# omerbt/Splice

Measured on AMD Instinct MI355X. Metric: opt_steps_per_sec, higher is better.
Workload: dtype bf16

## Files before the change

### splice_amd/csrc/step_engine.hip

```cpp
#include <memory>
#include <vector>

#include <stdio.h>
#include <stdlib.h>
#include <string.h>

#include "gen_kernels.h"
#include "kernels.h"
#include "optim.h"
#include "plateau.h"
#include "step_graph.h"

enum { L_TOTAL = 0, L_GLOBAL_SSIM = 1, L_ENTIRE_SSIM = 2, L_ENTIRE_CLS = 3, L_GLOBAL_CLS = 4, L_GLOBAL_ID = 5, L_TERMS = 6 };
enum { LAM_CLS = 0, LAM_SSIM = 1, LAM_ID = 2, LAM_ECLS = 3, LAM_ESSIM = 4 };
enum { PW_ESCALE_G = 0, PW_ESCALE_E = 1, PW_CLS = 2, PW_ID = 3, PW_ECLS = 4, PW_LAMBDAS = 5, PW_ROWS = 10 };
static const int TERM_LAM[L_TERMS] = {-1, LAM_SSIM, LAM_ESSIM, LAM_ECLS, LAM_CLS, LAM_ID};
static const int TERM_ROW[L_TERMS] = {-1, PW_ESCALE_G, PW_ESCALE_E, PW_ECLS, PW_CLS, PW_ID};

struct VitView {
    void* ctx = nullptr;
    int B = 0, H = 0, W = 0, D = 0, depth = 0, heads = 0, patch = 0, T = 0, Tld = 0, rows = 0;
    float* d_block = nullptr;
    float* d_keys = nullptr;
    float* imgs = nullptr;
    float* d_imgs = nullptr;
    std::vector<const float*> pb, pk;
};

struct SpliceStep {
    splice_step_config cfg;
    int P = 1;
    int Pa = 1, Pb = 1;
    int crops_mode = 0;
    int pairs = 1;
    int na = 1, nb = 1;
    size_t astride = 0;
    VitView vg, ve;
    void *plan_a = nullptr, *plan_b = nullptr, *plan_e = nullptr;
    int cropb_h = 0, cropb_w = 0;
    long long nparams = 0;
    float* gen_in = nullptr;
    float* in_b = nullptr;
    float* ent_in = nullptr;
    float* gen_out = nullptr;
    float* gen_out_b = nullptr;
    float *d_gen_out = nullptr, *d_gen_out_b = nullptr;
    float* ent_out = nullptr;
    float* d_ent_out = nullptr;
    void* ssim_ws = nullptr;
    float* losses = nullptr;
    size_t lp = 0, lstride = 0;
    std::vector<void*> allocs;
    int max_crop_h = 0, max_crop_w = 0;
    int* dev_t = nullptr;
    float* dev_lr = nullptr;
    int lr_set = 0;
    float lr = 0.f;
    int opt_kind = SPLICE_OPT_ADAM;
    float* pw = nullptr;
    float* pw_tab_alloc = nullptr;
    int pw_any[5] = {0, 0, 0, 0, 0};
    float* dev_lrs = nullptr;
    int pair_lr = 0;
    float lrs[SPLICE_STEP_MAX_PAIR_CFGS] = {};
    float opt_hp0 = 0.f, opt_hp1 = 0.f, opt_eps = 0.f;
    hipStream_t own_stream = nullptr;
    enum { EV_IN, EV_OUT, EV_FORK, EV_JOIN, EV_GB, EV_FORK2, EV_JOIN2, EV_KINDS };
    static constexpr int EV_RING = 4;
    hipEvent_t evs[EV_RING][EV_KINDS] = {};
    int ev_slot = 0;
    hipEvent_t ev(int kind) const { return evs[ev_slot][kind]; }
    hipStream_t side_stream = nullptr;
    int overlap = 1;
    int ablate = 0;
    StepGraphs graphs;
    void* graph_ptrs[6] = {nullptr, nullptr, nullptr, nullptr, nullptr, nullptr};
    float* losses_out = nullptr;
    int graph_crops[4] = {0, 0, 0, 0};
    float* grads_b = nullptr;
    int shape_repeats = 0;
    int repeat_step = -1;
    int use_graph = 1;
    int dbg_sync = 0;
    int ssim_id_on = 0;
    int skip_adam = 0, accumulate = 0;
    float* running = nullptr;
    long long running_stride = 0;
    int phases = 7;
    SpliceStep* leader = nullptr;
    splice_stop_state* stop = nullptr;
    StopRule stop_rule = {0, 0.f, 0, 0};
    int runs = 0;
};

static size_t arena_floats(const SpliceStep* st) { return st->astride ? st->pairs * st->astride : (size_t)st->nparams; }
static bool create_events(SpliceStep* st) {
    for (auto& set : st->evs)
        for (hipEvent_t& e : set)
            if (hipEventCreateWithFlags(&e, hipEventDisableTiming) != hipSuccess) return false;
    return true;
}

template <class T>
static int salloc(SpliceStep* st, T** p, size_t n) {
    void* q = nullptr;
    if (hipMalloc(&q, n * sizeof(T) + 256) != hipSuccess) {
        splice_set_error("splice_step: hipMalloc of %zu bytes failed", n * sizeof(T));
        return SPLICE_ERR_NOMEM;
    }
    st->allocs.push_back(q);
    *p = (T*)q;
    return SPLICE_OK;
}

static int view_init(SpliceStep* st, VitView& v, void* ctx, int want_B) {
    v.ctx = ctx;
    RC(splice_vit_ctx_dims(ctx, &v.B, &v.H, &v.W, &v.D, &v.depth, &v.heads, &v.patch));
    RC(splice_vit_ctx_info(ctx, &v.T, &v.Tld, &v.rows));
    RC(splice_vit_ctx_set_top_cls_only(ctx, st->cfg.top_cls_only));
    if (v.B != want_B) { splice_set_error("splice_step_create: ViT context has batch %d, need %d", v.B, want_B); return SPLICE_ERR_ARG; }
    RC(salloc(st, &v.d_block, (size_t)v.rows * v.D));
    RC(salloc(st, &v.d_keys, (size_t)v.rows * v.D));
    RC(salloc(st, &v.imgs, (size_t)v.B * 3 * v.H * v.W));
    RC(salloc(st, &v.d_imgs, (size_t)v.B * 3 * v.H * v.W));
    if (hipMemset(v.d_block, 0, (size_t)v.rows * v.D * sizeof(float)) != hipSuccess || hipMemset(v.d_keys, 0, (size_t)v.rows * v.D * sizeof(float)) != hipSuccess)
        return SPLICE_ERR_HIP;
    v.pb.assign(v.depth, nullptr);
    v.pk.assign(v.depth, nullptr);
    v.pb[v.depth - 1] = v.d_block;
    v.pk[v.depth - 1] = v.d_keys;
    return SPLICE_OK;
}

template <bool MONITOR>
__global__ __launch_bounds__(320) void total_loss_kernel(float* lbase, size_t lstride, int lp, float w_ssim, float w_essim, float w_ecls, float w_cls,
                                                         float w_id, float* out8, int n_a, int n_b, int n_c, int n_e, const float* wtab, int ssim_on,
                                                         int entire, splice_stop_state* stop, const int* dev_t, StopRule rule) {
    __shared__ float raw[8];
    float* l = lbase + (size_t)blockIdx.x * lstride;
    const int k = 1 + (threadIdx.x >> 6), lane = threadIdx.x & 63;
    const int n_slots = k == L_GLOBAL_SSIM ? n_a : k == L_GLOBAL_ID ? n_b : k == L_GLOBAL_CLS ? n_c : n_e;
    const float* lp0 = lbase + (size_t)blockIdx.x * n_slots * lstride;
    float tot = 0.f;
    for (int slot = 0; slot < n_slots; ++slot) {
        const float* part = lp0 + (size_t)slot * lstride + 8 + (size_t)k * lp;
        float acc = 0.f;
        for (int i = lane; i < lp; i += 64) acc += part[i];
        tot += wave_sum(acc);
    }
    const float acc = tot;
// ... 292 lines not shown
    const int P = st->P;
    for (int i = 0; i < 5 * P; ++i)
        if (!(lambdas[i] >= 0.f)) { splice_set_error("splice_step_set_pair_weights: lambdas must be >= 0"); return SPLICE_ERR_ARG; }
    std::vector<float> t((size_t)PW_ROWS * P, 0.f);
    const VitView &vg = st->vg, &ve = st->ve;
    const float ls_g = 1.0f / ((float)vg.T * (float)vg.T);
    const float ls_e = st->plan_e ? 1.0f / ((float)ve.T * (float)ve.T) : 0.f;
    const size_t n_cls = (size_t)1 * vg.D, n_id = (size_t)vg.T * vg.D, n_ecls = (size_t)1 * ve.D;
    for (int k = 0; k < 5; ++k) st->pw_any[k] = 0;
    for (int p = 0; p < P; ++p) {
        const float* l = lambdas + (size_t)p * 5;
        for (int k = 0; k < 5; ++k) st->pw_any[k] |= l[k] > 0.f;
        t[PW_ESCALE_G * P + p] = 4.0f * l[LAM_SSIM] * ls_g;
        if (st->plan_e) t[PW_ESCALE_E * P + p] = 4.0f * l[LAM_ESSIM] * ls_e;
        t[PW_CLS * P + p] = l[LAM_CLS] / (float)n_cls;
        t[PW_ID * P + p] = l[LAM_ID] / (float)n_id;
        if (st->plan_e) t[PW_ECLS * P + p] = l[LAM_ECLS] / (float)n_ecls;
        for (int k = 0; k < 5; ++k) t[PW_LAMBDAS * P + (size_t)p * 5 + k] = l[k];
    }
    st->graphs.retire();
    HIPCHK(hipDeviceSynchronize());
    HIPCHK(hipMemcpy(st->pw_tab_alloc, t.data(), t.size() * sizeof(float), hipMemcpyHostToDevice));
    st->pw = st->pw_tab_alloc;
    return SPLICE_OK;
}
int splice_step_set_pair_lr(void* h, const float* lr) {
    SpliceStep* st = (SpliceStep*)h;
    RC(pair_cfgs_ok(st, lr, "splice_step_set_pair_lr"));
    if (st->astride % 4) { splice_set_error("splice_step_set_pair_lr: the arena stride must be a multiple of 4"); return SPLICE_ERR_ARG; }
    if (!st->pair_lr) st->graphs.retire();
    st->pair_lr = 1;
    for (int p = 0; p < st->P; ++p) st->lrs[p] = lr[p];
    return SPLICE_OK;
}
int splice_step_set_phases(void* h, int phases, void* leader) {
    SpliceStep* st = (SpliceStep*)h;
    if (!st || phases <= 0 || phases > 7 || leader == h || (leader && phases != 2) || (leader && ((SpliceStep*)leader)->leader)) return SPLICE_ERR_ARG;
    if ((phases != 7 || leader) && st->stop_rule.window > 0) { splice_set_error("splice_step_set_phases: a handle with a stop rule runs whole steps (no phase mode)"); return SPLICE_ERR_STATE; }
    if (st->leader != (SpliceStep*)leader) st->graphs.retire();
    st->phases = phases;
    st->leader = (SpliceStep*)leader;
    return SPLICE_OK;
}

int splice_step_set_stop_rule(void* h, int window, float rel, int patience, int min_steps) {
    SpliceStep* st = (SpliceStep*)h;
    if (!st) return SPLICE_ERR_ARG;
    if (!stop_rule_ok(window, rel, patience, min_steps, "splice_step_set_stop_rule")) return SPLICE_ERR_ARG;
    if (st->runs > 0) { splice_set_error("splice_step_set_stop_rule: the rule is set before the first step"); return SPLICE_ERR_STATE; }
    if (st->skip_adam || st->phases != 7 || st->leader) {
        splice_set_error("splice_step_set_stop_rule: not on a handle in gradient-only (splice_step_set_mode) or phase mode (splice_step_set_phases)");
        return SPLICE_ERR_STATE;
    }
    if ((window > 0) != (st->stop_rule.window > 0)) st->graphs.retire();
    st->stop_rule = StopRule{window, rel, patience, min_steps};
    return SPLICE_OK;
}
int splice_step_stop_state(void* h, splice_stop_state* out, splice_stream_t stream) {
    SpliceStep* st = (SpliceStep*)h;
    if (!st || !out) return SPLICE_ERR_ARG;
    HIPCHK(hipMemcpyAsync(out, st->stop, (size_t)st->pairs * sizeof(splice_stop_state), hipMemcpyDeviceToHost, (hipStream_t)stream));
    HIPCHK(hipStreamSynchronize((hipStream_t)stream));
    return SPLICE_OK;
}
int splice_plateau_update(splice_stop_state* state, const float* losses8, int pairs, int window, float rel, int patience, int min_steps, int step_idx,
                          int counted, splice_stream_t stream) {
    if (!state || !losses8 || pairs < 1 || step_idx < 0) return SPLICE_ERR_ARG;
    if (!stop_rule_ok(window, rel, patience, min_steps, "splice_plateau_update")) return SPLICE_ERR_ARG;
    if (!counted || window == 0) return SPLICE_OK;
    SPLICE_LAUNCH(plateau_update_kernel, dim3((pairs + 63) / 64), dim3(64), 0, (hipStream_t)stream, state, losses8, pairs, StopRule{window, rel, patience, min_steps}, step_idx);
    return SPLICE_OK;
}

int splice_step_set_running_stats(void* h, float* running, long long stride) {
    SpliceStep* st = (SpliceStep*)h;
    if (!st || (running && st->P > 1 && stride <= 0)) return SPLICE_ERR_ARG;
    st->running = running; st->running_stride = stride;
    return SPLICE_OK;
}

static int place_passes(VitView& v, const float* src, int h, int w, int pass, int n, hipStream_t s) {
    return place_images(src, h, w, v.imgs + (size_t)pass * 3 * v.H * v.W, v.H, v.W, n, s);
}
static int zero_seeds(VitView& v, int pass, int n, hipStream_t s) {
    const size_t passD = (size_t)v.Tld * v.D;
    RC(dev_zero_launch(v.d_block + pass * passD, n * passD * sizeof(float), s));
    return dev_zero_launch(v.d_keys + pass * passD, n * passD * sizeof(float), s);
}

static int step_body(SpliceStep* st, float* params, float* grads, float* m, float* v, bool ssim_on, bool entire, hipStream_t s) {
    const splice_step_config& c = st->cfg;
    VitView &vg = st->vg, &ve = st->ve;
    const int P = st->P, Pa = st->Pa, Pb = st->Pb, pairs = st->pairs;
    const int nc = st->na < st->nb ? st->na : st->nb, Pc = pairs * nc;
    Term t[L_TERMS] = {};
    step_terms(st, ssim_on, entire, t);
    const StepPtrs ip = step_ptrs(st);
    const StepPtrs src = st->leader ? step_ptrs(st->leader) : ip;
    const bool do_gf = (st->phases & 1) != 0, do_v = (st->phases & 2) != 0, do_gb = (st->phases & 4) != 0;
    const bool gen_fwd = do_gf && !(st->ablate & 1), gen_bwd = do_gb && !(st->ablate & 2);
    auto chain_bwd = [&](VitView& vw, int p0, int p1, bool vit, float* d_img, int h, int w, float* d_lead, void* plan, float* arena, int accumulate,
                         bool gen, hipStream_t q) -> int {
        if (do_v) {
            if (vit) RC(splice_vit_backward(vw.ctx, p0, p1, vw.pb.data(), nullptr, vw.pk.data(), vw.d_imgs, 1, q));
            RC(unplace_grads(vw.d_imgs + (size_t)p0 * 3 * vw.H * vw.W, vw.H, vw.W, d_img, h, w, p1 - p0, q));
            if (st->leader) RC(add_f32_launch(d_lead, d_img, (size_t)(p1 - p0) * 3 * h * w, q));
        }
        if (gen) RC(splice_gen_backward(plan, params, d_img, arena, accumulate, q));
        return SPLICE_OK;
    };
    const int pA = 0, pB = Pa, pX = Pa + Pb, pY = 2 * Pa + Pb, pEnd = 2 * (Pa + Pb);
    const bool overlap = st->overlap && !splice_prof_active();
    hipStream_t s2 = overlap ? st->side_stream : s;
    if (overlap) {
        HIPCHK(hipEventRecord(st->ev(SpliceStep::EV_FORK), s));
        HIPCHK(hipStreamWaitEvent(s2, st->ev(SpliceStep::EV_FORK), 0));
    }
    if (gen_fwd) {
        RC(splice_gen_forward_borrowed(st->plan_b, params, src.b_in, ip.y, s2));
        if (overlap) HIPCHK(hipEventRecord(st->ev(SpliceStep::EV_GB), s2));
    }
    float *blk_g = nullptr, *qkv_g = nullptr;
    RC(splice_vit_get_tensor(vg.ctx, 0, vg.depth - 1, (void**)&blk_g));
    RC(splice_vit_get_tensor(vg.ctx, 3, vg.depth - 1, (void**)&qkv_g));
    const size_t passD = (size_t)vg.Tld * vg.D;
    SelfSimBatch sb = {};
    if (do_v) {
        RC(place_passes(vg, src.a_in, c.crop_h, c.crop_w, pA, Pa, s2));
        RC(place_passes(vg, src.b_in, st->cropb_h, st->cropb_w, pB, Pb, s2));
        if (!(st->ablate & 8)) RC(splice_vit_forward_passes(vg.ctx, vg.imgs, 1, pX, pA, pX, s2));
        RC(dev_zero_launch(st->losses, (size_t)P * st->lstride * sizeof(float), s2));
        RC(zero_seeds(vg, pX, Pa + Pb, s2));
        if (t[L_GLOBAL_SSIM].on) {
            RC(ssim_batch(st, vg, pA, pX, Pa, t[L_GLOBAL_SSIM], L_GLOBAL_SSIM, &sb));
            RC(selfsim_target_launch(sb, s2));
        }
    }
    if (overlap) HIPCHK(hipEventRecord(st->ev(SpliceStep::EV_JOIN), s2));
    if (gen_fwd) {
        RC(splice_gen_forward_borrowed(st->plan_a, params, src.a_in, ip.x, s));
        if (overlap) HIPCHK(hipStreamWaitEvent(s, st->ev(SpliceStep::EV_GB), 0));
    }
    if (do_v) {
        RC(place_passes(vg, src.x, c.crop_h, c.crop_w, pX, Pa, s));
        RC(place_passes(vg, src.y, st->cropb_h, st->cropb_w, pY, Pb, s));
        if (!(st->ablate & 16)) RC(splice_vit_forward_passes(vg.ctx, vg.imgs, 1, pX, pX, pEnd, s));
    }
    if (overlap) HIPCHK(hipStreamWaitEvent(s, st->ev(SpliceStep::EV_JOIN), 0));
    if (do_v) {
        if (t[L_GLOBAL_SSIM].on) RC(selfsim_loss_launch(sb, s));
        if (t[L_GLOBAL_CLS].on) {
            if (pairs > 1 && st->na != st->nb) {
                for (int i = 0; i < nc; ++i)
                    RC(mse_batched_launch(blk_g + (pX + i) * passD, vg.D, st->na * passD, blk_g + (pB + i) * passD, vg.D, st->nb * passD, 1, vg.D, 1.0f,
                                          t[L_GLOBAL_CLS].lambda, loss_part(st, L_GLOBAL_CLS) + (size_t)i * st->lstride, (size_t)nc * st->lstride,
                                          vg.d_block + (pX + i) * passD, vg.D, st->na * passD, pairs, s, nullptr));
            } else {
                RC(mse_batched_launch(blk_g + pX * passD, vg.D, passD, blk_g + pB * passD, vg.D, passD, 1, vg.D, 1.0f, t[L_GLOBAL_CLS].lambda,
                                      loss_part(st, L_GLOBAL_CLS), st->lstride, vg.d_block + pX * passD, vg.D, passD, Pc, s, t[L_GLOBAL_CLS].tab));
            }
        }
        if (t[L_GLOBAL_ID].on)
            RC(mse_batched_launch(keys_ptr(vg, qkv_g, pY), 3 * vg.D, 3 * passD, keys_ptr(vg, qkv_g, pB), 3 * vg.D, 3 * passD, vg.T, vg.D, 1.0f, t[L_GLOBAL_ID].lambda,
                                  loss_part(st, L_GLOBAL_ID), st->lstride, vg.d_keys + pY * passD, vg.D, passD, Pb, s, t[L_GLOBAL_ID].tab));
    }
    if (entire) {
        if (do_gf) RC(splice_gen_forward_borrowed(st->plan_e, params, src.e_in, ip.xe, s));
        if (do_v) {
            RC(place_passes(ve, src.e_in, c.ent_h, c.ent_w, 0, pairs, s));
            RC(place_passes(ve, src.xe, c.ent_h, c.ent_w, pairs, pairs, s));
            RC(splice_vit_forward_ex(ve.ctx, ve.imgs, 1, pairs, s));
            float* blk_e = nullptr;
            RC(splice_vit_get_tensor(ve.ctx, 0, ve.depth - 1, (void**)&blk_e));
            const size_t epassD = (size_t)ve.Tld * ve.D;
            RC(zero_seeds(ve, pairs, pairs, s));
            if (t[L_ENTIRE_SSIM].on) {
                SelfSimBatch se = {};
                RC(ssim_batch(st, ve, 0, pairs, pairs, t[L_ENTIRE_SSIM], L_ENTIRE_SSIM, &se));
                RC(selfsim_target_launch(se, s));
                RC(selfsim_loss_launch(se, s));
            }
            if (t[L_ENTIRE_CLS].on)
                RC(mse_batched_launch(blk_e + pairs * epassD, ve.D, epassD, blk_g + pB * passD, vg.D, st->nb * passD, 1, ve.D, 1.0f, t[L_ENTIRE_CLS].lambda,
                                      loss_part(st, L_ENTIRE_CLS), st->lstride, ve.d_block + pairs * epassD, ve.D, epassD, pairs, s, t[L_ENTIRE_CLS].tab));
        }
    }
    const bool stop_on = st->stop_rule.window > 0;
    auto bookkeeping = [&](hipStream_t q) -> int {
        if (do_v) {
            const bool grouped = st->crops_mode && pairs > 1;
            const int n1 = st->crops_mode ? P : 1;
            const auto kernel = stop_on ? total_loss_kernel<true> : total_loss_kernel<false>;
            SPLICE_LAUNCH(kernel, dim3(pairs), dim3(320), 0, q, st->losses, st->lstride, (int)st->lp, t[L_GLOBAL_SSIM].lambda, t[L_ENTIRE_SSIM].lambda,
                          t[L_ENTIRE_CLS].lambda, t[L_GLOBAL_CLS].lambda, t[L_GLOBAL_ID].lambda, st->losses_out, grouped ? st->na : n1, grouped ? st->nb : n1, grouped ? nc : n1,
                          grouped ? 1 : n1, st->pw ? st->pw + (size_t)PW_LAMBDAS * P : nullptr, (int)ssim_on, (int)entire, st->stop, st->dev_t, st->stop_rule);
        }
        if (!st->running || !gen_fwd) return SPLICE_OK;
        void* plans[3] = {st->plan_a, st->plan_b, nullptr};
        if (entire) { plans[1] = st->plan_e; plans[2] = st->plan_b; }
        return gen_running_stats_update(plans, entire ? 3 : 2, st->running, st->running_stride, 0.1f, stop_on ? st->stop : nullptr, st->dev_t, q);
    };
    const bool side_tail = overlap && !(st->ablate & 4);
    const float* adam_g2 = nullptr;
    if (!(st->ablate & 4)) {
        if (overlap) {
            HIPCHK(hipEventRecord(st->ev(SpliceStep::EV_FORK2), s));
            HIPCHK(hipStreamWaitEvent(s2, st->ev(SpliceStep::EV_FORK2), 0));
        }
        RC(chain_bwd(vg, pY, pEnd, !(st->ablate & 32), ip.dy, st->cropb_h, st->cropb_w, src.dy, st->plan_b, st->grads_b, 0, gen_bwd, s2));
        if (side_tail) {
            RC(bookkeeping(s2));
            HIPCHK(hipEventRecord(st->ev(SpliceStep::EV_JOIN2), s2));
        }
        RC(chain_bwd(vg, pX, pY, true, ip.dx, c.crop_h, c.crop_w, src.dx, st->plan_a, grads, st->accumulate, gen_bwd, s));
        if (overlap) HIPCHK(hipStreamWaitEvent(s, st->ev(SpliceStep::EV_JOIN2), 0));
        if (gen_bwd) {
            if (entire || st->skip_adam) RC(add_f32_launch(grads, st->grads_b, arena_floats(st), s));
            else adam_g2 = st->grads_b;
        }
    }
    if (entire) RC(chain_bwd(ve, pairs, 2 * pairs, true, ip.dxe, c.ent_h, c.ent_w, src.dxe, st->plan_e, grads, 1, do_gb, s));
    if (!side_tail) RC(bookkeeping(s));
    SPLICE_DEV_REGION(21);
    if (do_gb && !st->skip_adam) {
        OptimArgs a = {};
        a.kind = st->opt_kind; a.p = params; a.g = grads; a.g2 = adam_g2; a.m = m; a.v = v;
        a.n = arena_floats(st);
        a.lr = c.lr; a.hp0 = st->opt_hp0; a.hp1 = st->opt_hp1; a.eps = st->opt_eps; a.step_dev = st->dev_t;
        a.lr_dev = st->pair_lr ? st->dev_lrs : st->lr_set ? st->dev_lr : nullptr;
        a.lr_stride = st->pair_lr ? st->astride : 0;
        if (stop_on) { a.mask = st->stop; a.mask_step = st->dev_t; a.mask_stride = st->astride; }
        RC(optim_launch(a, s));
    }
    return SPLICE_OK;
}

int splice_step_run(void* h, float* params, float* grads, float* m, float* v, const float* A_crop, const float* B_crop,
                    const float* A_entire, int step_idx, float* losses_out, splice_stream_t stream) {
    SpliceStep* st = (SpliceStep*)h;
    if (!st || !params || !grads || !m || !v || !A_crop || !B_crop || step_idx < 0) return SPLICE_ERR_ARG;
#ifdef SPLICE_DEV_SWITCHES
    ++g_splice_dev_steps;
#endif
    hipStream_t caller = (hipStream_t)stream;
    const splice_step_config& c = st->cfg;
    const int P = st->P;
    st->ev_slot = (st->ev_slot + 1) % SpliceStep::EV_RING;
    ++st->runs;
    if (step_idx == c.cls_warmup) st->ssim_id_on = 1;
    const bool entire = c.ent_h > 0 && c.entire_every > 0 && (step_idx % c.entire_every == 0);
    if (entire && !A_entire) { splice_set_error("splice_step_run: step %d needs the entire structure image", step_idx); return SPLICE_ERR_ARG; }
    {
        void* ptrs[6] = {params, grads, m, v, losses_out, st->running};
        st->losses_out = losses_out;
        const int crops[4] = {c.crop_h, c.crop_w, st->cropb_h, st->cropb_w};
        if (memcmp(ptrs, st->graph_ptrs, sizeof(ptrs)) || memcmp(crops, st->graph_crops, sizeof(crops))) {
            st->graphs.retire();
            memcpy(st->graph_ptrs, ptrs, sizeof(ptrs));
            memcpy(st->graph_crops, crops, sizeof(crops));
            st->shape_repeats = 0;
            st->repeat_step = step_idx;
        } else if (step_idx != st->repeat_step) {
            if (st->shape_repeats < 2) ++st->shape_repeats;
            st->repeat_step = step_idx;
        }
    }
    const bool graph = st->use_graph && !splice_prof_active() && st->shape_repeats >= 2;
    hipStream_t s = caller;
    if (graph) {
        s = st->own_stream;
        HIPCHK(hipEventRecord(st->ev(SpliceStep::EV_IN), caller));
        HIPCHK(hipStreamWaitEvent(s, st->ev(SpliceStep::EV_IN), 0));
    }
    if (st->leader) {
        const SpliceStep* ld = st->leader;
        if (ld->P != P || ld->Pa != st->Pa || ld->Pb != st->Pb || ld->pairs != st->pairs || ld->cfg.crop_h != c.crop_h || ld->cfg.crop_w != c.crop_w ||
            ld->cropb_h != st->cropb_h || ld->cropb_w != st->cropb_w || ld->cfg.ent_h != c.ent_h || ld->cfg.ent_w != c.ent_w) {
            splice_set_error("splice_step_run: a follower's images must have the leader's shapes");
            return SPLICE_ERR_ARG;
        }
    }
    if (st->phases & 1) {
        StageArgs sa = {};
        const StepPtrs ip = step_ptrs(st);
        sa.src[0] = A_crop; sa.dst[0] = ip.a_in; sa.n[0] = (size_t)st->Pa * 3 * c.crop_h * c.crop_w;
        sa.src[1] = B_crop; sa.dst[1] = ip.b_in; sa.n[1] = (size_t)st->Pb * 3 * st->cropb_h * st->cropb_w;
        if (entire) { sa.src[2] = A_entire; sa.dst[2] = ip.e_in; sa.n[2] = (size_t)st->pairs * 3 * c.ent_h * c.ent_w; }
        sa.ip = st->dev_t; sa.iv = step_idx + 1;
        if (st->pair_lr) {
            sa.fp = st->dev_lrs; sa.nf = P;
            for (int p = 0; p < P; ++p) sa.fv[p] = st->lrs[p];
        } else if (st->lr_set) {
            sa.fp = st->dev_lr; sa.nf = 1; sa.fv[0] = st->lr;
        }
        SPLICE_LAUNCH(stage_inputs_kernel, dim3(128 * (P > 4 ? 4 : P)), dim3(256), 0, s, sa);
    }
    if (!graph) {
        RC(step_body(st, params, grads, m, v, st->ssim_id_on != 0, entire, s));
    } else {
        const int variant = (st->ssim_id_on ? 1 : 0) | (entire ? 2 : 0) | (st->phases << 2);
        hipGraphExec_t ex = st->graphs.find(variant);
        if (!ex) {
            hipGraph_t g = nullptr;
            HIPCHK(hipStreamBeginCapture(s, hipStreamCaptureModeThreadLocal));
// ... 47 lines not shown
```

### splice_amd/csrc/vit_engine.hip

```cpp
#include <string.h>

#include <string>
#include <vector>

#include "kernels.h"


struct Linear {
    bf16_t* w = nullptr;
    bf16_t* wT = nullptr;
    float* b = nullptr;
    int out = 0, in = 0;
    uint8_t* w8 = nullptr;
    float* w8_scale = nullptr;
};
struct LayerW {
    float *ln1_g = nullptr, *ln1_b = nullptr, *ln2_g = nullptr, *ln2_b = nullptr;
    Linear qkv, proj, fc1, fc2;
};

struct SpliceVit {
    int patch = 0, dim = 0, depth = 0, heads = 0, hidden = 0;
    int device = 0;
    std::vector<LayerW> layers;
// ... 14 lines not shown
    SpliceVit* vit = nullptr;
    int B = 0, H = 0, W = 0, T = 0, Tld = 0, rows = 0, need_grad = 0;
    int grad_pass_begin = 0;
    float* pos_eff = nullptr;
    bf16_t* patches = nullptr;
    std::vector<float*> xs;
    std::vector<float*> xmid;
    std::vector<float*> mean1, rstd1, mean2, rstd2;
    std::vector<bf16_t*> qkv, attn_out, hpre;
    bf16_t* qkvT_last = nullptr;
    std::vector<float*> lse;
    float* qkv_last_f32 = nullptr;
    bf16_t* ln_out = nullptr;
    int fp8 = 0;
    uint8_t* ln_out8 = nullptr;
    float* ln_scale = nullptr;
    uint8_t* hact8 = nullptr;
    uint8_t *qkv8 = nullptr, *qkvT8 = nullptr;
    bf16_t* hact = nullptr;
    float* g = nullptr;
    bf16_t* g_bf = nullptr;
    bf16_t* dh = nullptr;
    float* dln = nullptr;
    bf16_t *dout = nullptr, *dqkv = nullptr;
    float* delta = nullptr;
    float* dpatches = nullptr;
    std::vector<void*> allocs;
    int forward_done = 0;
    int top_cls_only = 0;
    bf16_t *cls_attn = nullptr, *cls_ln = nullptr, *cls_h = nullptr, *cls_dh = nullptr, *cls_dout = nullptr;
    float *cls_probs = nullptr, *cls_dln = nullptr;
    float* cls_slabs = nullptr;
};

template <class T>
static int dev_alloc(std::vector<void*>& list, T** p, size_t n) {
    void* q = nullptr;
    if (hipMalloc(&q, n * sizeof(T) + 256) != hipSuccess) {
        splice_set_error("hipMalloc of %zu bytes failed", n * sizeof(T));
        return SPLICE_ERR_NOMEM;
    }
    list.push_back(q);
    *p = (T*)q;
    return SPLICE_OK;
}

static int pack_linear(SpliceVit* v, Linear& L, const float* w, int out, int in, hipStream_t s) {
    L.out = out; L.in = in;
    RC(dev_alloc(v->allocs, &L.w, (size_t)out * in));
    RC(dev_alloc(v->allocs, &L.wT, (size_t)out * in));
    RC(cast_f32_bf16_launch(w, L.w, (size_t)out * in, s));
    RC(transpose_f32_to_bf16_launch(w, L.wT, out, in, out, s));
    return SPLICE_OK;
}
__global__ void scale_f32_kernel(float* dst, const float* src, size_t n, size_t n_scaled, float f) {
    for (size_t i = (size_t)blockIdx.x * blockDim.x + threadIdx.x; i < n; i += (size_t)gridDim.x * blockDim.x) dst[i] = i < n_scaled ? src[i] * f : src[i];
}
static int pack_qkv(SpliceVit* v, Linear& L, const float* w, int D, hipStream_t s) {
    if (!v->qfold) return pack_linear(v, L, w, 3 * D, D, s);
    float* tmp = nullptr;
    const size_t n = (size_t)3 * D * D;
    HIPCHK(hipMalloc((void**)&tmp, n * sizeof(float)));
    hipLaunchKernelGGL(scale_f32_kernel, dim3(1024), dim3(256), 0, s, tmp, w, n, (size_t)D * D, v->qscale);
    const int rc = pack_linear(v, L, tmp, 3 * D, D, s);
    (void)hipStreamSynchronize(s);
    (void)hipFree(tmp);
    return rc;
}
static int copy_vec(SpliceVit* v, float** dst, const float* src, size_t n, hipStream_t s) {
    RC(dev_alloc(v->allocs, dst, n));
    HIPCHK(hipMemcpyAsync(*dst, src, n * sizeof(float), hipMemcpyDeviceToDevice, s));
    return SPLICE_OK;
}

__global__ void add_f32_into_bf16_kernel(bf16_t* dst, int ldd, int col0, const float* src, int lds, int rows, int cols, int qcols, float qf) {
    const size_t n = (size_t)rows * cols;
    for (size_t i = (size_t)blockIdx.x * blockDim.x + threadIdx.x; i < n; i += (size_t)gridDim.x * blockDim.x) {
        const int r = i / cols, c = i % cols;
        bf16_t* p = dst + (size_t)r * ldd + col0 + c;
        const float v = src[(size_t)r * lds + c];
        *p = f2bf(bf2f(*p) + (c < qcols ? v * qf : v));
    }
}
__global__ void grad_stream_kernel(float* g, bf16_t* g_bf, const float* add, size_t n, int init) {
    for (size_t i = (size_t)blockIdx.x * blockDim.x + threadIdx.x; i < n; i += (size_t)gridDim.x * blockDim.x) {
        float v = init ? 0.f : g[i];
        if (add) v += add[i];
        g[i] = v;
        g_bf[i] = f2bf(v);
    }
}
__global__ void scale_cols_bf16_kernel(bf16_t* x, int ld, int rows, int cols, float f) {
    const size_t n = (size_t)rows * cols;
    for (size_t i = (size_t)blockIdx.x * blockDim.x + threadIdx.x; i < n; i += (size_t)gridDim.x * blockDim.x) {
        bf16_t* p = x + (i / cols) * ld + i % cols;
        *p = f2bf(bf2f(*p) * f);
    }
}
__global__ void scale_cols_f32_kernel(float* x, int ld, int rows, int cols, float f) {
    const size_t n = (size_t)rows * cols;
    for (size_t i = (size_t)blockIdx.x * blockDim.x + threadIdx.x; i < n; i += (size_t)gridDim.x * blockDim.x) x[(i / cols) * ld + i % cols] *= f;
}
static inline unsigned grid_n(size_t n) { size_t b = (n + 255) / 256; return (unsigned)(b > 2048 ? 2048 : (b ? b : 1)); }

extern "C" {

int splice_vit_create(int patch, int dim, int depth, int heads, void** out) {
    if (!out || (patch != 8 && patch != 16) || dim % 64 || dim / 64 != heads || depth < 1 || dim > 1024) {
        splice_set_error("splice_vit_create: unsupported config patch=%d dim=%d depth=%d heads=%d (head dim must be 64)", patch, dim, depth, heads);
        return SPLICE_ERR_ARG;
    }
    SpliceVit* v = new SpliceVit();
    v->patch = patch; v->dim = dim; v->depth = depth; v->heads = heads; v->hidden = 4 * dim;
    v->qfold = 1;
    v->qscale = v->qfold ? 0.125f * kLog2e : 1.0f;
    (void)hipGetDevice(&v->device);
    v->layers.resize(depth);
    *out = v;
    return SPLICE_OK;
}

void splice_vit_destroy(void* h) {
    SpliceVit* v = (SpliceVit*)h;
    if (!v) return;
    for (void* p : v->allocs) (void)hipFree(p);
    delete v;
}

int splice_vit_set_param(void* h, const char* name, const float* data, long long numel, splice_stream_t stream) {
    SpliceVit* v = (SpliceVit*)h;
    hipStream_t s = (hipStream_t)stream;
    if (!v || !name || !data) return SPLICE_ERR_ARG;
    const int D = v->dim, Hd = v->hidden, pp3 = 3 * v->patch * v->patch;
    std::string n(name);
    auto expect = [&](long long want) {
        if (numel != want) { splice_set_error("splice_vit_set_param(%s): numel %lld, expected %lld", name, numel, want); return false; }
        return true;
    };
    if (n == "cls_token") { if (!expect(D)) return SPLICE_ERR_ARG; RC(copy_vec(v, &v->cls, data, D, s)); }
    else if (n == "pos_embed") {
        if (numel % D) return SPLICE_ERR_ARG;
        v->pos_tokens = (int)(numel / D);
        RC(copy_vec(v, &v->pos, data, numel, s));
    }
    else if (n == "patch_embed.proj.weight") { if (!expect((long long)D * pp3)) return SPLICE_ERR_ARG; RC(pack_linear(v, v->pe, data, D, pp3, s)); }
    else if (n == "patch_embed.proj.bias") { if (!expect(D)) return SPLICE_ERR_ARG; RC(copy_vec(v, &v->pe.b, data, D, s)); }
    else if (n == "norm.weight") { if (!expect(D)) return SPLICE_ERR_ARG; RC(copy_vec(v, &v->norm_g, data, D, s)); }
    else if (n == "norm.bias") { if (!expect(D)) return SPLICE_ERR_ARG; RC(copy_vec(v, &v->norm_b, data, D, s)); }
    else if (n.rfind("blocks.", 0) == 0) {
        const size_t dot = n.find('.', 7);
        if (dot == std::string::npos) return SPLICE_ERR_ARG;
        const int li = atoi(n.substr(7, dot - 7).c_str());
        if (li < 0 || li >= v->depth) { splice_set_error("splice_vit_set_param: layer %d out of range", li); return SPLICE_ERR_ARG; }
        LayerW& L = v->layers[li];
        const std::string r = n.substr(dot + 1);
        if (r == "norm1.weight") { if (!expect(D)) return SPLICE_ERR_ARG; RC(copy_vec(v, &L.ln1_g, data, D, s)); }
        else if (r == "norm1.bias") { if (!expect(D)) return SPLICE_ERR_ARG; RC(copy_vec(v, &L.ln1_b, data, D, s)); }
        else if (r == "norm2.weight") { if (!expect(D)) return SPLICE_ERR_ARG; RC(copy_vec(v, &L.ln2_g, data, D, s)); }
        else if (r == "norm2.bias") { if (!expect(D)) return SPLICE_ERR_ARG; RC(copy_vec(v, &L.ln2_b, data, D, s)); }
        else if (r == "attn.qkv.weight") { if (!expect(3LL * D * D)) return SPLICE_ERR_ARG; RC(pack_qkv(v, L.qkv, data, D, s)); }
        else if (r == "attn.qkv.bias") { if (!expect(3 * D)) return SPLICE_ERR_ARG; RC(copy_vec(v, &L.qkv.b, data, 3 * D, s)); if (v->qfold) hipLaunchKernelGGL(scale_f32_kernel, dim3(8), dim3(256), 0, s, L.qkv.b, L.qkv.b, (size_t)3 * D, (size_t)D, v->qscale); }
        else if (r == "attn.proj.weight") { if (!expect((long long)D * D)) return SPLICE_ERR_ARG; RC(pack_linear(v, L.proj, data, D, D, s)); }
        else if (r == "attn.proj.bias") { if (!expect(D)) return SPLICE_ERR_ARG; RC(copy_vec(v, &L.proj.b, data, D, s)); }
        else if (r == "mlp.fc1.weight") { if (!expect((long long)Hd * D)) return SPLICE_ERR_ARG; RC(pack_linear(v, L.fc1, data, Hd, D, s)); }
        else if (r == "mlp.fc1.bias") { if (!expect(Hd)) return SPLICE_ERR_ARG; RC(copy_vec(v, &L.fc1.b, data, Hd, s)); }
        else if (r == "mlp.fc2.weight") { if (!expect((long long)Hd * D)) return SPLICE_ERR_ARG; RC(pack_linear(v, L.fc2, data, D, Hd, s)); }
// ... 284 lines not shown
                RC(gemm_nt_launch(EPI_BIAS | EPI_GELU | EPI_OUT_BF, ln_out, D, W.fc1.w, D, R, Hd, D, e, s));
            }
        }
        {
            GemmEpi e = {};
            e.bias = W.fc2.b; e.resid = x_mid; e.ldr = D; e.out_f32 = c->xs[l + 1] + r0 * D; e.ldo = D;
            SpliceProfScope ps(4); SPLICE_DEV_REGION(6);
            if (fp8) {
                e.row_scale = nullptr; e.col_scale = W.fc2.w8_scale;
                RC(gemm_nt_fp8_launch(EPI_SCALE_RC | EPI_BIAS | EPI_RESID | EPI_OUT_F32, c->hact8 + r0 * Hd, Hd, W.fc2.w8, Hd, R, D, Hd, e, s));
            } else {
                RC(gemm_nt_launch(EPI_BIAS | EPI_RESID | EPI_OUT_F32, hact, Hd, W.fc2.w, Hd, R, D, Hd, e, s));
            }
        }
    }
    c->forward_done = 1;
    const hipError_t e = hipGetLastError();
    if (e != hipSuccess) { splice_set_error("splice_vit_forward: %s", hipGetErrorString(e)); return SPLICE_ERR_HIP; }
    return SPLICE_OK;
}

int splice_vit_get_tensor(void* ctx, int kind, int layer, void** out) {
    SpliceVitCtx* c = (SpliceVitCtx*)ctx;
    if (!c || !out || layer < 0 || layer >= c->vit->depth) return SPLICE_ERR_ARG;
    switch (kind) {
        case 0: *out = c->xs[layer + 1]; break;
        case 1: *out = c->qkv[layer]; break;
        case 2: *out = c->attn_out[layer]; break;
        case 3: *out = c->qkv_last_f32; break;
        case 4: *out = c->lse[layer]; break;
        case 5: *out = c->xs[0]; break;
        case 6: if (layer != c->vit->depth - 1) return SPLICE_ERR_ARG; *out = c->qkvT_last; break;
        case 7: *out = c->qkv[layer]; break;
        default: return SPLICE_ERR_ARG;
    }
    return SPLICE_OK;
}

int splice_vit_read_tensor(void* ctx, int kind, int layer, void* dst, size_t bytes, splice_stream_t stream) {
    void* src = nullptr;
    RC(splice_vit_get_tensor(ctx, kind, layer, &src));
    HIPCHK(hipMemcpyAsync(dst, src, bytes, hipMemcpyDeviceToDevice, (hipStream_t)stream));
    SpliceVitCtx* c = (SpliceVitCtx*)ctx;
    if (c->vit->qfold && (kind == 1 || kind == 3)) {
        const int D = c->vit->dim;
        const size_t rows = bytes / ((size_t)3 * D * (kind == 1 ? 2 : 4));
        if (kind == 1) hipLaunchKernelGGL(scale_cols_bf16_kernel, dim3(grid_n(rows * D)), dim3(256), 0, (hipStream_t)stream, (bf16_t*)dst, 3 * D, (int)rows, D, 1.0f / c->vit->qscale);
        else hipLaunchKernelGGL(scale_cols_f32_kernel, dim3(grid_n(rows * D)), dim3(256), 0, (hipStream_t)stream, (float*)dst, 3 * D, (int)rows, D, 1.0f / c->vit->qscale);
    }
    return SPLICE_OK;
}

int splice_vit_backward(void* ctx, int pass_begin, int pass_end, const float* const* d_block, const float* const* d_qkv,
                        const float* const* d_keys, float* d_img, int normalize, splice_stream_t stream) {
    SpliceVitCtx* c = (SpliceVitCtx*)ctx;
    if (!c || !c->need_grad || !c->forward_done || pass_begin < c->grad_pass_begin || pass_end > c->B || pass_begin >= pass_end || !d_img) {
        splice_set_error("splice_vit_backward: bad ctx / range / no forward / ctx created without need_grad");
        return SPLICE_ERR_STATE;
    }
    SpliceVit* v = c->vit;
    hipStream_t s = (hipStream_t)stream;
    const int D = v->dim, Hd = v->hidden, pp3 = 3 * v->patch * v->patch, L = v->depth;
    const size_t r0 = (size_t)pass_begin * c->Tld;
    const int R = (pass_end - pass_begin) * c->Tld;
    const int Bp = pass_end - pass_begin;
    float* g = c->g + r0 * D;
    bf16_t* g_bf = c->g_bf + r0 * D;
    bool g_live = false;
    const size_t slab = (size_t)c->rows * D;
    const int tiles1 = cdiv(c->Tld, 64) * cdiv(D, 64);
    const int ks = (tiles1 * 3 <= 640 && D % 192 == 0) ? 3 : (tiles1 <= 640 && D % 128 == 0) ? 2 : 1;
    for (int l = L - 1; l >= 0; --l) {
        const LayerW& W = v->layers[l];
        const float* db = d_block ? d_block[l] : nullptr;
        const float* dq = d_qkv ? d_qkv[l] : nullptr;
        const float* dk = d_keys ? d_keys[l] : nullptr;
        if (db) {
            SPLICE_LAUNCH(grad_stream_kernel, dim3(grid_n((size_t)R * D)), dim3(256), 0, s, g, g_bf, db + r0 * D, (size_t)R * D, g_live ? 0 : 1);
            g_live = true;
        }
        if (!g_live && !dq && !dk) continue;
        bf16_t* dqkv = c->dqkv + r0 * 3 * D;
        const float* g_after_mlp = nullptr;
        if (g_live && l == L - 1 && c->top_cls_only) {
            SPLICE_DEV_REGION(20);
            const int rs = c->Tld * D, hs = c->Tld * Hd;
            bf16_t* cdh = c->cls_dh + (size_t)pass_begin * Hd;
            const size_t sstr = (size_t)c->B * Hd;
            float* slabs = c->cls_slabs + (size_t)pass_begin * Hd;
            auto ks_of = [](int K) { int n = K / 64, k = 16; while (k > 1 && n % k) --k; return k; };
            {
                GemmEpi e = {};
                e.out_f32 = slabs; e.ldo = Hd; e.ksplit = ks_of(D); e.slab_stride = (long long)sstr;
                RC(gemm_nt_launch(EPI_OUT_F32, g_bf, rs, W.fc2.wT, D, Bp, Hd, D, e, s));
                RC(rows_finish_launch(2, slabs, e.ksplit, sstr, Bp, Hd, nullptr, nullptr, 0, nullptr, 0, cdh, nullptr, c->hpre[l] + r0 * Hd, hs, 0, s));
            }
            {
                GemmEpi e = {};
                e.out_f32 = slabs; e.ldo = D; e.ksplit = ks_of(Hd); e.slab_stride = (long long)sstr;
                RC(gemm_nt_launch(EPI_OUT_F32, cdh, Hd, W.fc1.wT, Hd, Bp, D, Hd, e, s));
                RC(ln_rows_bwd_launch(slabs, D, c->xmid[l] + r0 * D, rs, W.ln2_g, c->mean2[l] + r0, c->rstd2[l] + r0, c->Tld, g, g_bf, Bp, D, e.ksplit, sstr, s));
            }
            {
                GemmEpi e = {};
                e.out_f32 = slabs; e.ldo = D; e.ksplit = ks_of(D); e.slab_stride = (long long)sstr;
                RC(gemm_nt_launch(EPI_OUT_F32, g_bf, rs, W.proj.wT, D, Bp, D, D, e, s));
                RC(attn_cls_bwd_launch(c->qkv[l] + r0 * 3 * D, c->qkvT_last + r0, c->rows, Bp, c->T, c->Tld, D, v->heads, v->qfold ? kLn2 : 0.125f,
                                       c->cls_probs + (size_t)pass_begin * v->heads * c->Tld, slabs, e.ksplit, sstr, dqkv, s));
            }
            g_after_mlp = g;
        } else if (g_live) {
            {
                GemmEpi e = {};
                e.aux = c->hpre[l] + r0 * Hd; e.ldaux = Hd; e.out_bf = c->dh + r0 * Hd; e.ldbf = Hd;
                SpliceProfScope ps(11); SPLICE_DEV_REGION(7);
                RC(gemm_nt_launch(EPI_GELU_GRAD | EPI_OUT_BF, g_bf, D, W.fc2.wT, D, R, Hd, D, e, s));
            }
            {
                GemmEpi e = {};
                e.out_f32 = c->dln + r0 * D; e.ldo = D; e.ksplit = ks; e.slab_stride = (long long)slab;
                SpliceProfScope ps(5); SPLICE_DEV_REGION(8);
                RC(gemm_nt_launch(EPI_OUT_F32, c->dh + r0 * Hd, Hd, W.fc1.wT, Hd, R, D, Hd, e, s));
            }
            {
                SpliceProfScope ps(10); SPLICE_DEV_REGION(9);
                RC(layernorm_bwd_slabs_launch(c->dln + r0 * D, gemm_splitk_slabs(R, ks), slab, c->xmid[l] + r0 * D, W.ln2_g, c->mean2[l] + r0, c->rstd2[l] + r0, g, g, g_bf, R, D, s));
            }
            {
                GemmEpi e = {};
                e.out_bf = c->dout + r0 * D; e.ldbf = D;
                e.rd_other = c->attn_out[l] + r0 * D; e.ld_rd = D; e.rd_rows = c->Tld;
                e.rowdot = c->delta + (size_t)pass_begin * v->heads * c->Tld;
                SpliceProfScope ps(11); SPLICE_DEV_REGION(10);
                RC(gemm_nt_launch(EPI_OUT_BF | EPI_ROWDOT, g_bf, D, W.proj.wT, D, R, D, D, e, s));
            }
            {
                AttnArgs a = {};
                a.qkv = c->qkv[l] + r0 * 3 * D; a.B = Bp; a.T = c->T; a.Tld = c->Tld;
                a.D = D; a.H = v->heads; a.scale = v->qfold ? kLn2 : 0.125f; a.qfold = v->qfold; a.out = c->attn_out[l] + r0 * D;
                a.lse = c->lse[l] + (size_t)pass_begin * v->heads * c->Tld;
                a.dout = c->dout + r0 * D; a.doutT = nullptr; a.delta = c->delta + (size_t)pass_begin * v->heads * c->Tld; a.delta_ready = 1; a.dqkv = dqkv;
                SpliceProfScope ps(6); SPLICE_DEV_REGION(11);
                RC(attn_bwd_launch(&a, s));
            }
            g_after_mlp = g;
        } else {
            RC(dev_zero_launch(dqkv, (size_t)R * 3 * D * sizeof(bf16_t), s));
        }
        if (dq) SPLICE_LAUNCH(add_f32_into_bf16_kernel, dim3(grid_n((size_t)R * 3 * D)), dim3(256), 0, s, dqkv, 3 * D, 0, dq + r0 * 3 * D, 3 * D, R, 3 * D, v->qfold ? D : 0, 1.0f / v->qscale);
        if (dk) SPLICE_LAUNCH(add_f32_into_bf16_kernel, dim3(grid_n((size_t)R * D)), dim3(256), 0, s, dqkv, 3 * D, D, dk + r0 * D, D, R, D, 0, 1.0f);
        {
            GemmEpi e = {};
            e.out_f32 = c->dln + r0 * D; e.ldo = D; e.ksplit = ks; e.slab_stride = (long long)slab;
            SpliceProfScope ps(5); SPLICE_DEV_REGION(12);
            RC(gemm_nt_launch(EPI_OUT_F32, dqkv, 3 * D, W.qkv.wT, 3 * D, R, D, 3 * D, e, s));
        }
        {
            SpliceProfScope ps(10); SPLICE_DEV_REGION(9);
            RC(layernorm_bwd_slabs_launch(c->dln + r0 * D, gemm_splitk_slabs(R, ks), slab, c->xs[l] + r0 * D, W.ln1_g, c->mean1[l] + r0, c->rstd1[l] + r0, g_after_mlp, g, g_bf, R, D, s));
        }
        g_live = true;
    }
    if (!g_live) {
        RC(dev_zero_launch(d_img + (size_t)pass_begin * 3 * c->H * c->W, (size_t)Bp * 3 * c->H * c->W * sizeof(float), s));
        return SPLICE_OK;
    }
    {
        GemmEpi e = {};
        e.out_f32 = c->dpatches + r0 * pp3; e.ldo = pp3;
        RC(gemm_nt_launch(EPI_OUT_F32, g_bf, D, v->pe.wT, D, R, pp3, D, e, s));
    }
    RC(unpatchify_launch(c->dpatches + r0 * pp3, d_img + (size_t)pass_begin * 3 * c->H * c->W, Bp, c->H, c->W, v->patch, c->Tld, normalize, s));
    const hipError_t e = hipGetLastError();
    if (e != hipSuccess) { splice_set_error("splice_vit_backward: %s", hipGetErrorString(e)); return SPLICE_ERR_HIP; }
    return SPLICE_OK;
}
}
```

Measured before the change: 262.8.

## Run key-loss backward chain on side stream and skip dead block/qkv grad work

Moves the global identity (keys) MSE loss launch and the pY..pEnd ViT backward chain onto the side stream, forking right after the forward join so it overlaps the CLS/SSIM losses. It also drops the block-output seed for those passes and stops zeroing their block seeds. When only the key gradient is live, it writes only the key window of dqkv instead of zeroing the whole buffer, and runs a K=D GEMM against the key slice of the qkv weights rather than a split-K 3D GEMM. The risks are ordering hazards on the shared losses buffer (guarded by the EV_LOSS event) and the key_window path relying on ks==3 and a single-slab layout.

After: 264.7 (median of 6 runs). No clear change (+0.7%).

```diff
diff --git a/splice_amd/csrc/step_engine.hip b/splice_amd/csrc/step_engine.hip
--- a/splice_amd/csrc/step_engine.hip
+++ b/splice_amd/csrc/step_engine.hip
@@ -65,7 +65,7 @@
     float lrs[SPLICE_STEP_MAX_PAIR_CFGS] = {};
     float opt_hp0 = 0.f, opt_hp1 = 0.f, opt_eps = 0.f;
     hipStream_t own_stream = nullptr;
-    enum { EV_IN, EV_OUT, EV_FORK, EV_JOIN, EV_GB, EV_FORK2, EV_JOIN2, EV_KINDS };
+    enum { EV_IN, EV_OUT, EV_FORK, EV_JOIN, EV_GB, EV_FORK2, EV_LOSS, EV_JOIN2, EV_KINDS };
     static constexpr int EV_RING = 4;
     hipEvent_t evs[EV_RING][EV_KINDS] = {};
     int ev_slot = 0;
@@ -524,10 +524,10 @@
 static int place_passes(VitView& v, const float* src, int h, int w, int pass, int n, hipStream_t s) {
     return place_images(src, h, w, v.imgs + (size_t)pass * 3 * v.H * v.W, v.H, v.W, n, s);
 }
-static int zero_seeds(VitView& v, int pass, int n, hipStream_t s) {
+static int zero_seeds(VitView& v, int pass, int n_block, int n_keys, hipStream_t s) {
     const size_t passD = (size_t)v.Tld * v.D;
-    RC(dev_zero_launch(v.d_block + pass * passD, n * passD * sizeof(float), s));
-    return dev_zero_launch(v.d_keys + pass * passD, n * passD * sizeof(float), s);
+    RC(dev_zero_launch(v.d_block + pass * passD, n_block * passD * sizeof(float), s));
+    return dev_zero_launch(v.d_keys + pass * passD, n_keys * passD * sizeof(float), s);
 }
 
 static int step_body(SpliceStep* st, float* params, float* grads, float* m, float* v, bool ssim_on, bool entire, hipStream_t s) {
@@ -541,10 +541,10 @@
     const StepPtrs src = st->leader ? step_ptrs(st->leader) : ip;
     const bool do_gf = (st->phases & 1) != 0, do_v = (st->phases & 2) != 0, do_gb = (st->phases & 4) != 0;
     const bool gen_fwd = do_gf && !(st->ablate & 1), gen_bwd = do_gb && !(st->ablate & 2);
-    auto chain_bwd = [&](VitView& vw, int p0, int p1, bool vit, float* d_img, int h, int w, float* d_lead, void* plan, float* arena, int accumulate,
+    auto chain_bwd = [&](VitView& vw, int p0, int p1, bool vit, bool block_seed, float* d_img, int h, int w, float* d_lead, void* plan, float* arena, int accumulate,
                          bool gen, hipStream_t q) -> int {
         if (do_v) {
-            if (vit) RC(splice_vit_backward(vw.ctx, p0, p1, vw.pb.data(), nullptr, vw.pk.data(), vw.d_imgs, 1, q));
+            if (vit) RC(splice_vit_backward(vw.ctx, p0, p1, block_seed ? vw.pb.data() : nullptr, nullptr, vw.pk.data(), vw.d_imgs, 1, q));
             RC(unplace_grads(vw.d_imgs + (size_t)p0 * 3 * vw.H * vw.W, vw.H, vw.W, d_img, h, w, p1 - p0, q));
             if (st->leader) RC(add_f32_launch(d_lead, d_img, (size_t)(p1 - p0) * 3 * h * w, q));
         }
@@ -572,7 +572,7 @@
         RC(place_passes(vg, src.b_in, st->cropb_h, st->cropb_w, pB, Pb, s2));
         if (!(st->ablate & 8)) RC(splice_vit_forward_passes(vg.ctx, vg.imgs, 1, pX, pA, pX, s2));
         RC(dev_zero_launch(st->losses, (size_t)P * st->lstride * sizeof(float), s2));
-        RC(zero_seeds(vg, pX, Pa + Pb, s2));
+        RC(zero_seeds(vg, pX, Pa, Pa + Pb, s2));
         if (t[L_GLOBAL_SSIM].on) {
             RC(ssim_batch(st, vg, pA, pX, Pa, t[L_GLOBAL_SSIM], L_GLOBAL_SSIM, &sb));
             RC(selfsim_target_launch(sb, s2));
@@ -589,6 +589,15 @@
         if (!(st->ablate & 16)) RC(splice_vit_forward_passes(vg.ctx, vg.imgs, 1, pX, pX, pEnd, s));
     }
     if (overlap) HIPCHK(hipStreamWaitEvent(s, st->ev(SpliceStep::EV_JOIN), 0));
+    const bool side_chain = overlap && !(st->ablate & 4);
+    hipStream_t sy = side_chain ? s2 : s;
+    if (side_chain) {
+        HIPCHK(hipEventRecord(st->ev(SpliceStep::EV_FORK2), s));
+        HIPCHK(hipStreamWaitEvent(s2, st->ev(SpliceStep::EV_FORK2), 0));
+    }
+    if (do_v && t[L_GLOBAL_ID].on)
+        RC(mse_batched_launch(keys_ptr(vg, qkv_g, pY), 3 * vg.D, 3 * passD, keys_ptr(vg, qkv_g, pB), 3 * vg.D, 3 * passD, vg.T, vg.D, 1.0f, t[L_GLOBAL_ID].lambda,
+                              loss_part(st, L_GLOBAL_ID), st->lstride, vg.d_keys + pY * passD, vg.D, passD, Pb, sy, t[L_GLOBAL_ID].tab));
     if (do_v) {
         if (t[L_GLOBAL_SSIM].on) RC(selfsim_loss_launch(sb, s));
         if (t[L_GLOBAL_CLS].on) {
@@ -602,9 +611,6 @@
                                       loss_part(st, L_GLOBAL_CLS), st->lstride, vg.d_block + pX * passD, vg.D, passD, Pc, s, t[L_GLOBAL_CLS].tab));
             }
         }
-        if (t[L_GLOBAL_ID].on)
-            RC(mse_batched_launch(keys_ptr(vg, qkv_g, pY), 3 * vg.D, 3 * passD, keys_ptr(vg, qkv_g, pB), 3 * vg.D, 3 * passD, vg.T, vg.D, 1.0f, t[L_GLOBAL_ID].lambda,
-                                  loss_part(st, L_GLOBAL_ID), st->lstride, vg.d_keys + pY * passD, vg.D, passD, Pb, s, t[L_GLOBAL_ID].tab));
     }
     if (entire) {
         if (do_gf) RC(splice_gen_forward_borrowed(st->plan_e, params, src.e_in, ip.xe, s));
@@ -615,7 +621,7 @@
             float* blk_e = nullptr;
             RC(splice_vit_get_tensor(ve.ctx, 0, ve.depth - 1, (void**)&blk_e));
             const size_t epassD = (size_t)ve.Tld * ve.D;
-            RC(zero_seeds(ve, pairs, pairs, s));
+            RC(zero_seeds(ve, pairs, pairs, pairs, s));
             if (t[L_ENTIRE_SSIM].on) {
                 SelfSimBatch se = {};
                 RC(ssim_batch(st, ve, 0, pairs, pairs, t[L_ENTIRE_SSIM], L_ENTIRE_SSIM, &se));
@@ -642,26 +648,24 @@
         if (entire) { plans[1] = st->plan_e; plans[2] = st->plan_b; }
         return gen_running_stats_update(plans, entire ? 3 : 2, st->running, st->running_stride, 0.1f, stop_on ? st->stop : nullptr, st->dev_t, q);
     };
-    const bool side_tail = overlap && !(st->ablate & 4);
+    const bool side_tail = side_chain;
     const float* adam_g2 = nullptr;
     if (!(st->ablate & 4)) {
-        if (overlap) {
-            HIPCHK(hipEventRecord(st->ev(SpliceStep::EV_FORK2), s));
-            HIPCHK(hipStreamWaitEvent(s2, st->ev(SpliceStep::EV_FORK2), 0));
-        }
-        RC(chain_bwd(vg, pY, pEnd, !(st->ablate & 32), ip.dy, st->cropb_h, st->cropb_w, src.dy, st->plan_b, st->grads_b, 0, gen_bwd, s2));
+        if (side_tail) HIPCHK(hipEventRecord(st->ev(SpliceStep::EV_LOSS), s));
+        RC(chain_bwd(vg, pY, pEnd, !(st->ablate & 32), false, ip.dy, st->cropb_h, st->cropb_w, src.dy, st->plan_b, st->grads_b, 0, gen_bwd, sy));
         if (side_tail) {
+            HIPCHK(hipStreamWaitEvent(s2, st->ev(SpliceStep::EV_LOSS), 0));
             RC(bookkeeping(s2));
             HIPCHK(hipEventRecord(st->ev(SpliceStep::EV_JOIN2), s2));
         }
-        RC(chain_bwd(vg, pX, pY, true, ip.dx, c.crop_h, c.crop_w, src.dx, st->plan_a, grads, st->accumulate, gen_bwd, s));
+        RC(chain_bwd(vg, pX, pY, true, true, ip.dx, c.crop_h, c.crop_w, src.dx, st->plan_a, grads, st->accumulate, gen_bwd, s));
         if (overlap) HIPCHK(hipStreamWaitEvent(s, st->ev(SpliceStep::EV_JOIN2), 0));
         if (gen_bwd) {
             if (entire || st->skip_adam) RC(add_f32_launch(grads, st->grads_b, arena_floats(st), s));
             else adam_g2 = st->grads_b;
         }
     }
-    if (entire) RC(chain_bwd(ve, pairs, 2 * pairs, true, ip.dxe, c.ent_h, c.ent_w, src.dxe, st->plan_e, grads, 1, do_gb, s));
+    if (entire) RC(chain_bwd(ve, pairs, 2 * pairs, true, true, ip.dxe, c.ent_h, c.ent_w, src.dxe, st->plan_e, grads, 1, do_gb, s));
     if (!side_tail) RC(bookkeeping(s));
     SPLICE_DEV_REGION(21);
     if (do_gb && !st->skip_adam) {
diff --git a/splice_amd/csrc/vit_engine.hip b/splice_amd/csrc/vit_engine.hip
--- a/splice_amd/csrc/vit_engine.hip
+++ b/splice_amd/csrc/vit_engine.hip
@@ -120,6 +120,13 @@
         *p = f2bf(bf2f(*p) + (c < qcols ? v * qf : v));
     }
 }
+__global__ void set_bf16_window_kernel(bf16_t* dst, int ldd, int col0, const float* src, int rows, int cols, int Tld, int T) {
+    const size_t n = (size_t)rows * cols;
+    for (size_t i = (size_t)blockIdx.x * blockDim.x + threadIdx.x; i < n; i += (size_t)gridDim.x * blockDim.x) {
+        const int r = i / cols, c = i % cols;
+        dst[(size_t)r * ldd + col0 + c] = f2bf(r % Tld < T ? 0.f + src[i] : 0.f);
+    }
+}
 __global__ void grad_stream_kernel(float* g, bf16_t* g_bf, const float* add, size_t n, int init) {
     for (size_t i = (size_t)blockIdx.x * blockDim.x + threadIdx.x; i < n; i += (size_t)gridDim.x * blockDim.x) {
         float v = init ? 0.f : g[i];
@@ -570,6 +577,7 @@
         if (!g_live && !dq && !dk) continue;
         bf16_t* dqkv = c->dqkv + r0 * 3 * D;
         const float* g_after_mlp = nullptr;
+        const bool key_window = !g_live && !dq && dk && ks == 3;
         if (g_live && l == L - 1 && c->top_cls_only) {
             SPLICE_DEV_REGION(20);
             const int rs = c->Tld * D, hs = c->Tld * Hd;
@@ -632,20 +640,29 @@
                 RC(attn_bwd_launch(&a, s));
             }
             g_after_mlp = g;
+        } else if (key_window) {
         } else {
             RC(dev_zero_launch(dqkv, (size_t)R * 3 * D * sizeof(bf16_t), s));
         }
         if (dq) SPLICE_LAUNCH(add_f32_into_bf16_kernel, dim3(grid_n((size_t)R * 3 * D)), dim3(256), 0, s, dqkv, 3 * D, 0, dq + r0 * 3 * D, 3 * D, R, 3 * D, v->qfold ? D : 0, 1.0f / v->qscale);
-        if (dk) SPLICE_LAUNCH(add_f32_into_bf16_kernel, dim3(grid_n((size_t)R * D)), dim3(256), 0, s, dqkv, 3 * D, D, dk + r0 * D, D, R, D, 0, 1.0f);
+        if (key_window) SPLICE_LAUNCH(set_bf16_window_kernel, dim3(grid_n((size_t)R * D)), dim3(256), 0, s, dqkv, 3 * D, D, dk + r0 * D, R, D, c->Tld, c->T);
+        else if (dk) SPLICE_LAUNCH(add_f32_into_bf16_kernel, dim3(grid_n((size_t)R * D)), dim3(256), 0, s, dqkv, 3 * D, D, dk + r0 * D, D, R, D, 0, 1.0f);
+        int n_slabs = gemm_splitk_slabs(R, ks);
         {
             GemmEpi e = {};
-            e.out_f32 = c->dln + r0 * D; e.ldo = D; e.ksplit = ks; e.slab_stride = (long long)slab;
+            e.out_f32 = c->dln + r0 * D; e.ldo = D;
             SpliceProfScope ps(5); SPLICE_DEV_REGION(12);
-            RC(gemm_nt_launch(EPI_OUT_F32, dqkv, 3 * D, W.qkv.wT, 3 * D, R, D, 3 * D, e, s));
+            if (key_window) {
+                n_slabs = 1;
+                RC(gemm_nt_launch(EPI_OUT_F32, dqkv + D, 3 * D, W.qkv.wT + D, 3 * D, R, D, D, e, s));
+            } else {
+                e.ksplit = ks; e.slab_stride = (long long)slab;
+                RC(gemm_nt_launch(EPI_OUT_F32, dqkv, 3 * D, W.qkv.wT, 3 * D, R, D, 3 * D, e, s));
+            }
         }
         {
             SpliceProfScope ps(10); SPLICE_DEV_REGION(9);
-            RC(layernorm_bwd_slabs_launch(c->dln + r0 * D, gemm_splitk_slabs(R, ks), slab, c->xs[l] + r0 * D, W.ln1_g, c->mean1[l] + r0, c->rstd1[l] + r0, g_after_mlp, g, g_bf, R, D, s));
+            RC(layernorm_bwd_slabs_launch(c->dln + r0 * D, n_slabs, slab, c->xs[l] + r0 * D, W.ln1_g, c->mean1[l] + r0, c->rstd1[l] + r0, g_after_mlp, g, g_bf, R, D, s));
         }
         g_live = true;
     }
```
